# Asunatan/LM-Net

Hardware: AMD Instinct MI355X
Metric: train images/sec at 352x352, 1/2/4/8 MI355X; Dice vs ref (higher is better)
Workload: dtype f32; 1 GPU; LM-Net fp32 training step (fwd + CE/Dice loss + bwd + AdamW), batch 8/GPU, 352x352 synthetic disc masks (BASELINE configs[1]); global_batch=8, parallelism=dp1, launch=lmn_plan_run (recorded C-side schedule, one crossing per pass)

## Files before the change

lm_net_amd/csrc/conv_wgrad.hip:

```cpp
#include "conv_common.h"

namespace {

struct WgradParams {
  LmnLay lay_src[3], lay_dy;
  int32_t rpw;
  uint32_t rp_magic;
  lmn_wgrad_args_t a;
  int ntile_src[3];
  int ntile_off[3];
  int cbase[3];
  int NNTT, NMTT;
  int Cin;
  int nsets_n;
  int steps_per_img;
  int total_steps;
  float inv_keep_src[3];
  float inv_keep_dy;
  float* partial;
  int TH, TW, XH, XW, CSx, CSy, tiles_x, tiles_y, total_tiles;
  uint32_t mXW, mTW;
  int dbg;
};

__device__ __forceinline__ float* wgrad_dst(const WgradParams& P, int co, int sidx, int ch, int taps) {
  float* own = P.a.dW_src[sidx];
  return own ? own + ((int64_t)co * P.a.src[sidx].C + ch) * taps
             : P.a.dW + ((int64_t)co * P.Cin + P.cbase[sidx] + ch) * taps;
}

template <int TAPS, int NMT, int NNT, int PM = 0>
__global__ __launch_bounds__(256, 2) void wgrad_lds_kernel(const WgradParams P) {
  constexpr bool BF = PM >= 1;
  typedef typename ActT<PM>::type TA;
  const lmn_wgrad_args_t& A = P.a;
  const uint32_t soff = A.seed_ctr ? *A.seed_ctr : 0u;
  extern __shared__ __attribute__((aligned(16))) float smem[];
  const int XP = P.XH * P.XW;
  float* XS = smem;
  float* YS = smem + NNT * XP * P.CSx;
  const int tid = threadIdx.x, lane = tid & 63;
  const int wv = __builtin_amdgcn_readfirstlane(tid >> 6);
  const int q = lane >> 4, n = lane & 15;
  const int mset = blockIdx.y / P.nsets_n, nset = blockIdx.y - mset * P.nsets_n;
  const int mt0 = mset * NMT, nt0 = nset * NNT;
  const int pad = A.ksize >> 1;
  const int NP = P.TH * P.TW;

  const TA* tptr[NNT];
  const float* tscale[NNT];
  int tC[NNT], tcs[NNT], tflags[NNT], tch0[NNT];
  uint32_t tseed[NNT];
  float tp_[NNT], tik[NNT];
#pragma unroll
  for (int t = 0; t < NNT; ++t) {
    const int nt = nt0 + t;
    int sidx = 0;
    while (sidx + 1 < A.nsrc && nt >= P.ntile_off[sidx + 1]) ++sidx;
    tptr[t] = (const TA*)A.src[sidx].ptr;
    tscale[t] = A.src[sidx].scale;
    tC[t] = nt < P.NNTT ? A.src[sidx].C : 0;
    tcs[t] = A.src[sidx].cstride;
    tflags[t] = A.src[sidx].flags;
    tseed[t] = A.src[sidx].drop_seed + soff;
    tp_[t] = A.src[sidx].drop_p;
    tik[t] = P.inv_keep_src[sidx];
    tch0[t] = (nt - P.ntile_off[sidx]) * 16;
  }

  f32x4 acc[TAPS][NMT][NNT];
  float bsum[NMT];
#pragma unroll
  for (int tp = 0; tp < TAPS; ++tp)
#pragma unroll
    for (int m = 0; m < NMT; ++m)
#pragma unroll
      for (int t = 0; t < NNT; ++t) acc[tp][m][t] = f32x4{0.f, 0.f, 0.f, 0.f};
#pragma unroll
  for (int m = 0; m < NMT; ++m) bsum[m] = 0.f;

  const int t_begin = (int)(((int64_t)blockIdx.x * P.total_tiles) / gridDim.x);
  const int t_end = (int)(((int64_t)(blockIdx.x + 1) * P.total_tiles) / gridDim.x);
  for (int tile = t_begin; tile < t_end; ++tile) {
    const int b = tile / (P.tiles_x * P.tiles_y), tt = tile - b * P.tiles_x * P.tiles_y;
    const int oy0 = (tt / P.tiles_x) * P.TH, ox0 = (tt % P.tiles_x) * P.TW;
    const int iy0 = oy0 * A.stride - pad, ix0 = ox0 * A.stride - pad;
    __syncthreads();
    constexpr int UX = (TAPS == 9 && NMT * NNT == 4) ? 3 : 4, UY = 2;
    const int NXI = P.XH * P.XW * 4, NYI = NP * 4;
    for (int rd = 0; rd * (UX * 256) < NXI || rd * (UY * 256) < NYI; ++rd) {
      f32x4 vx[UX][NNT], vy[UY][NMT];
      int gpx[UX], gpy[UY];
#pragma unroll
      for (int u = 0; u < UX; ++u) {
        const int i = rd * (UX * 256) + u * 256 + tid;
        const int j = i & 3, pix = i >> 2;
        bool inb;
        int gp;
        if constexpr (TAPS == 1) {
          inb = i < NXI && ox0 + pix < A.Wout;
          gp = inb ? b * A.Wout + ox0 + pix : 0;
        } else {
          const int r = (int)__umulhi((uint32_t)pix, P.mXW), c = pix - r * P.XW;
          const int iy = iy0 + r, ix = ix0 + c;
          inb = i < NXI && (unsigned)iy < (unsigned)A.Hin && (unsigned)ix < (unsigned)A.Win;
          gp = inb ? (b * A.Hin + iy) * A.Win + ix : 0;
// ... 179 lines not shown
            for (int r = 0; r < 4; ++r) {
              float* d = &s_acc[(((tp * NMT + m) * NNT + t) * 4 + r) * 64 + lane];
              *d = (w == 0) ? acc[tp][m][t][r] : *d + acc[tp][m][t][r];
            }
#pragma unroll
      for (int m = 0; m < NMT; ++m) {
        float v = bsum[m];
        v += __shfl_xor(v, 16, 64);
        v += __shfl_xor(v, 32, 64);
        if (q == 0) {
          float* d = &s_acc[NT * 256 + m * 16 + n];
          *d = (w == 0) ? v : *d + v;
        }
      }
    }
    __syncthreads();
  }
  if (P.partial) {
    float* dst = P.partial + ((int64_t)blockIdx.y * gridDim.x + blockIdx.x) * (NT * 256 + NMT * 16);
    for (int i = tid; i < NT * 256 + NMT * 16; i += 256) dst[i] = s_acc[i];
    return;
  }
  for (int i = tid; i < NT * 256; i += 256) {
    const int ln = i & 63, r = (i >> 6) & 3, tl = i >> 8;
    const int t = tl % NNT, m = (tl / NNT) % NMT, tp = tl / (NNT * NMT);
    const int qq = ln >> 4, nn = ln & 15;
    const int co = (mt0 + m) * 16 + qq * 4 + r;
    const int nt = nt0 + t;
    if ((mt0 + m) >= P.NMTT || co >= A.Cout || nt >= P.NNTT) continue;
    int sidx = 0;
    while (sidx + 1 < A.nsrc && nt >= P.ntile_off[sidx + 1]) ++sidx;
    const int ch = (nt - P.ntile_off[sidx]) * 16 + nn;
    if (ch >= A.src[sidx].C) continue;
    atomicAdd(wgrad_dst(P, co, sidx, ch, TAPS) + tp, s_acc[i]);
  }
  if (A.db && nset == 0) {
    for (int i = tid; i < NMT * 16; i += 256) {
      const int co = mt0 * 16 + i;
      if (co < A.Cout && (mt0 + i / 16) < P.NMTT) {
        atomicAdd(A.db + co, s_acc[NT * 256 + i]);
        if (A.db2) atomicAdd(A.db2 + co, s_acc[NT * 256 + i]);
      }
    }
  }
}

template <int ESZ> struct RawOf { typedef f32x4 type; };
template <> struct RawOf<2> { typedef u32x2 type; };
__device__ __forceinline__ f32x4 raw_f32(f32x4 v) { return v; }
__device__ __forceinline__ f32x4 raw_f32(u32x2 v) { return f32x4{lmn_bf16_lo(v.x), lmn_bf16_hi(v.x), lmn_bf16_lo(v.y), lmn_bf16_hi(v.y)}; }
template <typename RawT> __device__ __forceinline__ RawT raw_load(BufRsrc r, uint32_t off) {
  if constexpr (sizeof(RawT) == 16) return __builtin_bit_cast(f32x4, __builtin_amdgcn_raw_buffer_load_b128(r, (int)off, 0, 0));
  else return __builtin_amdgcn_raw_buffer_load_b64(r, (int)off, 0, 0);
}
#ifdef LMN_WG_TIMING
__device__ unsigned long long g_wg_timing[4096 * 6];
#define LMN_TCLK() __builtin_amdgcn_s_memtime()
#endif

template <int NMT, int NNT, int PM, bool UP = false>
__global__ __launch_bounds__(256, 3) void wgrad3_kernel(const WgradParams P) {
  static_assert(NMT * NNT == 4 || NMT * NNT == 1, "one-tile or 2 x 2-tile blocks");
  constexpr bool TS = NMT * NNT == 4;
  constexpr bool BF = PM >= 1;
  typedef typename ActT<PM>::type TA;
  constexpr int ESZ = sizeof(TA);
  typedef typename RawOf<ESZ>::type RawT;
  constexpr int XWC = 34, CS = BF ? 12 : 16;
  constexpr int QW = BF ? 2 : 4;
  constexpr int UX = TS ? 4 : 6, UY = TS ? 2 : 4;
  constexpr int XPA = UX * 64, NPA = UY * 64;
  const lmn_wgrad_args_t& A = P.a;
  const uint32_t soff = A.seed_ctr ? *A.seed_ctr : 0u;
  extern __shared__ __attribute__((aligned(16))) float smem[];
  float* XS = smem;
  float* YS = smem + NNT * XPA * CS;
  constexpr int USX = TS ? 2 : 3;
  constexpr int SCW = 19, SPA = USX * 64;
  float* S2 = YS + NMT * NPA * CS;
  (void)S2;
  const int tid = threadIdx.x, lane = tid & 63;
  const int wv = __builtin_amdgcn_readfirstlane(tid >> 6);
  const int q = lane >> 4, n = lane & 15;
  const int m_w = TS ? wv / NNT : 0, t_w = TS ? wv % NNT : 0;
  const int mset = blockIdx.y / P.nsets_n, nset = blockIdx.y - mset * P.nsets_n;
  const int mt0 = mset * NMT, nt0 = nset * NNT;
  const int NP = P.TH * 32;
  const int j = tid & 3, pl = tid >> 2;

  const float* tscale[NNT];
  int tC[NNT], tcs[NNT], tflags[NNT], tch0[NNT];
  uint32_t tseed[NNT];
  float tp_[NNT], tik[NNT];
  BufRsrc rx[NNT];
  bool cx[NNT];
#pragma unroll
  for (int t = 0; t < NNT; ++t) {
    const int nt = nt0 + t;
    int sidx = 0;
    while (sidx + 1 < A.nsrc && nt >= P.ntile_off[sidx + 1]) ++sidx;
    tscale[t] = A.src[sidx].scale;
    tC[t] = nt < P.NNTT ? A.src[sidx].C : 0;
    tcs[t] = A.src[sidx].cstride;
    tflags[t] = A.src[sidx].flags;
    tseed[t] = A.src[sidx].drop_seed + soff;
    tp_[t] = A.src[sidx].drop_p;
    tik[t] = P.inv_keep_src[sidx];
    tch0[t] = (nt - P.ntile_off[sidx]) * 16;
    rx[t] = make_rsrc(A.src[sidx].ptr, (unsigned)((int64_t)A.B * (UP ? (A.Hin >> 1) * (A.Win >> 1) : A.Hin * A.Win) * tcs[t] * ESZ));
    cx[t] = tch0[t] + j * 4 < tC[t];
  }
  const BufRsrc ry = make_rsrc(A.dy, (unsigned)((int64_t)A.B * A.Hout * A.Wout * A.dy_cstride * ESZ));

  uint32_t xrc[UX], xo[UX][NNT];
#pragma unroll
  for (int u = 0; u < UX; ++u) {
    const int pix = u * 64 + pl, r = pix / XWC, c = pix - r * XWC;
    xrc[u] = r < P.XH ? (uint32_t)(r << 16 | c) : 0x7fff0000u;
#pragma unroll
    for (int t = 0; t < NNT; ++t) xo[u][t] = (uint32_t)(((r * A.Win + c) * tcs[t] + tch0[t] + j * 4) * ESZ);
  }
  const int yc = pl & 31, yr0 = pl >> 5;
  uint32_t yo0[NMT];
  bool cy[NMT];
#pragma unroll
  for (int m = 0; m < NMT; ++m) {
    const int co = (mt0 + m) * 16 + j * 4;
    cy[m] = (mt0 + m) < P.NMTT && co < A.Cout;
    yo0[m] = (uint32_t)(((yr0 * A.Wout + yc) * A.dy_cstride + (cy[m] ? co : 0)) * ESZ);
  }
  const uint32_t ystep = (uint32_t)(2 * A.Wout * A.dy_cstride * ESZ);

  f32x4 acc[9];
  float bsum = 0.f;
#pragma unroll
  for (int tp = 0; tp < 9; ++tp) acc[tp] = f32x4{0.f, 0.f, 0.f, 0.f};

  RawT vx[UP ? 1 : UX][NNT], vy[UY][NMT];
  RawT vs[UP ? USX : 1][NNT];
  const int tpi = P.tiles_x * P.tiles_y;
  const int hs = A.Hin >> 1, ws = A.Win >> 1;
  const float up_sh = UP ? (float)(hs - 1) / (float)(A.Hin - 1) : 0.f, up_sw = UP ? (float)(ws - 1) / (float)(A.Win - 1) : 0.f;
  auto src_org = [&](int iy0, int ix0, int& ys0, int& xs0) __attribute__((always_inline)) {
    ys0 = (int)(up_sh * (float)(iy0 > 0 ? iy0 : 0));
    xs0 = (int)(up_sw * (float)(ix0 > 0 ? ix0 : 0));
  };
  auto issue = [&](int tile) __attribute__((always_inline)) {
    const int b = tile / tpi, tt = tile - b * tpi;
    const int ty_ = tt / P.tiles_x;
    const int oy0 = ty_ * P.TH, ox0 = (tt - ty_ * P.tiles_x) * 32;
    const int iy0 = oy0 - 1, ix0 = ox0 - 1;
    const int wpix = (b * A.Hin + iy0) * A.Win + ix0;
    if constexpr (UP) {
      int ys0, xs0;
      src_org(iy0, ix0, ys0, xs0);
#pragma unroll
      for (int u = 0; u < USX; ++u) {
        const int sp = u * 64 + pl, sr = sp / SCW, sc = sp - sr * SCW;
        const bool inb = ys0 + sr < hs && xs0 + sc < ws;
#pragma unroll
        for (int t = 0; t < NNT; ++t) {
          const uint32_t off = (uint32_t)((((b * hs + ys0 + sr) * ws + xs0 + sc) * tcs[t] + tch0[t] + j * 4) * ESZ);
          vs[u][t] = raw_load<RawT>(rx[t], (inb && cx[t]) ? off : 0xffffffffu);
        }
      }
    } else {
#pragma unroll
    for (int u = 0; u < UX; ++u) {
      const int r = (int)(xrc[u] >> 16), c = (int)(xrc[u] & 0xffffu);
      const bool inb = (unsigned)(iy0 + r) < (unsigned)A.Hin && (unsigned)(ix0 + c) < (unsigned)A.Win;
#pragma unroll
      for (int t = 0; t < NNT; ++t) {
        const uint32_t off = (uint32_t)(wpix * tcs[t] * ESZ) + xo[u][t];
        vx[u][t] = raw_load<RawT>(rx[t], (inb && cx[t]) ? off : 0xffffffffu);
      }
    }
    }
    const uint32_t ybase = (uint32_t)(((b * A.Hout + oy0) * A.Wout + ox0) * A.dy_cstride * ESZ);
    const bool cok = ox0 + yc < A.Wout;
    const int rlim = (A.Hout - oy0 < P.TH ? A.Hout - oy0 : P.TH) - yr0;
#pragma unroll
    for (int u = 0; u < UY; ++u) {
      const bool inb = cok && 2 * u < rlim;
#pragma unroll
      for (int m = 0; m < NMT; ++m)
        vy[u][m] = raw_load<RawT>(ry, (inb && cy[m]) ? ybase + (uint32_t)u * ystep + yo0[m] : 0xffffffffu);
    }
  };
  float* xl = XS + pl * CS + j * QW;
  float* yl = YS + pl * CS + j * QW;
  auto commit = [&](int tile) __attribute__((always_inline)) {
    const int b = tile / tpi, tt = tile - b * tpi;
    const int ty_ = tt / P.tiles_x;
    const int oy0 = ty_ * P.TH, ox0 = (tt - ty_ * P.tiles_x) * 32;
    if constexpr (UP) {
#pragma unroll
      for (int t = 0; t < NNT; ++t)
#pragma unroll
        for (int u = 0; u < USX; ++u) *reinterpret_cast<f32x4*>(&S2[((t * SPA) + u * 64 + pl) * 16 + j * 4]) = raw_f32(vs[u][t]);
      __syncthreads();
      const int iy0 = oy0 - 1, ix0 = ox0 - 1;
      int ys0, xs0;
      src_org(iy0, ix0, ys0, xs0);
#pragma unroll
      for (int u = 0; u < UX; ++u) {
        const int r = (int)(xrc[u] >> 16), c = (int)(xrc[u] & 0xffffu);
        const int iy = iy0 + r, ix = ix0 + c;
        const bool inb = (unsigned)iy < (unsigned)A.Hin && (unsigned)ix < (unsigned)A.Win;
        int y0, yp, x0, xp;
        float ly0, ly1, lx0, lx1;
        lmn_up_coord(inb ? iy : 0, hs, up_sh, y0, yp, ly0, ly1);
        lmn_up_coord(inb ? ix : 0, ws, up_sw, x0, xp, lx0, lx1);
        const int l00 = inb ? (y0 - ys0) * SCW + (x0 - xs0) : 0;
#pragma unroll
        for (int t = 0; t < NNT; ++t) {
          const float* sp = &S2[(t * SPA + l00) * 16 + j * 4];
          const f32x4 v00 = *reinterpret_cast<const f32x4*>(sp), v01 = *reinterpret_cast<const f32x4*>(sp + xp * 16);
          const f32x4 v10 = *reinterpret_cast<const f32x4*>(sp + yp * SCW * 16), v11 = *reinterpret_cast<const f32x4*>(sp + (yp * SCW + xp) * 16);
          f32x4 w = ly0 * (lx0 * v00 + lx1 * v01) + ly1 * (lx0 * v10 + lx1 * v11);
          if (!inb) w = f32x4{0.f, 0.f, 0.f, 0.f};
          float* dst = xl + (t * XPA + u * 64) * CS;
          if constexpr (BF) *reinterpret_cast<uint2*>(dst) = pk4_bf16(w);
          else *reinterpret_cast<f32x4*>(dst) = w;
        }
      }
    } else {
#pragma unroll
    for (int t = 0; t < NNT; ++t) {
      const bool tf = tflags[t] != 0 || tscale[t] != nullptr;
#pragma unroll
      for (int u = 0; u < UX; ++u) {
        float* dst = xl + (t * XPA + u * 64) * CS;
        if (!tf) {
          if constexpr (ESZ == 2) *reinterpret_cast<u32x2*>(dst) = vx[u][t];
          else if constexpr (BF) *reinterpret_cast<uint2*>(dst) = pk4_bf16(raw_f32(vx[u][t]));
          else *reinterpret_cast<f32x4*>(dst) = raw_f32(vx[u][t]);
          continue;
        }
        f32x4 w = raw_f32(vx[u][t]);
        const int chs = cx[t] ? tch0[t] + j * 4 : 0;
        if (tflags[t] & LMN_SRC_GELU) {
#pragma unroll
          for (int k = 0; k < 4; ++k) w[k] = lmn_gelu(w[k]);
        }
        if (tflags[t] & LMN_SRC_DROP) {
          const int r = (int)(xrc[u] >> 16), c = (int)(xrc[u] & 0xffffu);
          const int gp = (b * A.Hin + oy0 - 1 + r) * A.Win + ox0 - 1 + c;
#pragma unroll
          for (int k = 0; k < 4; ++k) w[k] *= lmn_drop_scale(tseed[t], (uint32_t)(gp * tC[t] + chs + k), tp_[t], tik[t]);
        }
        if (tscale[t]) w *= ld4(tscale[t] + b * tC[t] + chs);
        if constexpr (BF) *reinterpret_cast<uint2*>(dst) = pk4_bf16(w);
        else *reinterpret_cast<f32x4*>(dst) = w;
      }
    }
    }
#pragma unroll
    for (int m = 0; m < NMT; ++m) {
#pragma unroll
      for (int u = 0; u < UY; ++u) {
        float* dst = yl + (m * NPA + u * 64) * CS;
        if (!(A.dy_flags & LMN_SRC_DROP)) {
          if constexpr (ESZ == 2) *reinterpret_cast<u32x2*>(dst) = vy[u][m];
          else if constexpr (BF) *reinterpret_cast<uint2*>(dst) = pk4_bf16(raw_f32(vy[u][m]));
          else *reinterpret_cast<f32x4*>(dst) = raw_f32(vy[u][m]);
          continue;
        }
        f32x4 w = raw_f32(vy[u][m]);
        const int cos = cy[m] ? (mt0 + m) * 16 + j * 4 : 0;
        const int gp = (b * A.Hout + oy0 + 2 * u + yr0) * A.Wout + ox0 + yc;
#pragma unroll
        for (int k = 0; k < 4; ++k) w[k] *= lmn_drop_scale(A.dy_seed + soff, (uint32_t)(gp * A.Cout + cos + k), A.dy_p, P.inv_keep_dy);
        if constexpr (BF) *reinterpret_cast<uint2*>(dst) = pk4_bf16(w);
        else *reinterpret_cast<f32x4*>(dst) = w;
      }
    }
  };

  const int t_begin = (int)(((int64_t)blockIdx.x * P.total_tiles) / gridDim.x);
  const int t_end = (int)(((int64_t)(blockIdx.x + 1) * P.total_tiles) / gridDim.x);
#ifdef LMN_WG_TIMING
  unsigned long long tk0 = LMN_TCLK(), tk_s1 = 0, tk_s2 = 0, tk_s3 = 0, tk_a, tk_b;
#endif
  if (t_begin < t_end) issue(t_begin);
  const int K0 = TS ? 0 : wv, KSTEP = TS ? 1 : 4;
  for (int tile = t_begin; tile < t_end; ++tile) {
#ifdef LMN_WG_TIMING
    tk_a = LMN_TCLK();
#endif
    __syncthreads();
#ifdef LMN_WG_TIMING
    tk_b = LMN_TCLK(); tk_s1 += tk_b - tk_a; tk_a = tk_b;
#endif
    commit(tile);
#ifdef LMN_WG_TIMING
    __builtin_amdgcn_s_waitcnt(0);
    tk_b = LMN_TCLK(); tk_s2 += tk_b - tk_a; tk_a = tk_b;
#endif
    __syncthreads();
    if (tile + 1 < t_end) issue(tile + 1);
#ifdef LMN_WG_TIMING
    tk_b = LMN_TCLK(); tk_s3 += tk_b - tk_a;
#endif
    if constexpr (BF) {
      const uint16_t* xw = reinterpret_cast<const uint16_t*>(XS) + (t_w * XPA + q * 4) * (CS * 2) + n;
      const uint16_t* yw = reinterpret_cast<const uint16_t*>(YS) + (m_w * NPA + q * 4) * (CS * 2) + n;
      auto kfrag = [&](int ks, uint2& av, uint2 (&bv)[9]) __attribute__((always_inline)) {
        const int pix0 = ks * 16, pr = pix0 >> 5, pc0 = pix0 & 31;
        const uint16_t* xp = xw + (pr * XWC + pc0) * (CS * 2);
        const uint16_t* yp = yw + pix0 * (CS * 2);
        uint32_t h[4];
#pragma unroll
        for (int jj = 0; jj < 4; ++jj) {
          h[jj] = yp[jj * CS * 2];
          bsum += __builtin_bit_cast(float, h[jj] << 16);
        }
        av = uint2{h[0] | (h[1] << 16), h[2] | (h[3] << 16)};
#pragma unroll
        for (int tp = 0; tp < 9; ++tp) {
          const uint16_t* xt = xp + ((tp / 3) * XWC + tp % 3) * (CS * 2);
          const uint32_t h0 = xt[0], h1 = xt[CS * 2], h2 = xt[2 * CS * 2], h3 = xt[3 * CS * 2];
          bv[tp] = uint2{h0 | (h1 << 16), h2 | (h3 << 16)};
        }
      };
      int ks = K0;
      for (; (ks + KSTEP) * 16 < NP; ks += 2 * KSTEP) {
        uint2 av0, av1, bv0[9], bv1[9];
        kfrag(ks, av0, bv0);
        kfrag(ks + KSTEP, av1, bv1);
#pragma unroll
        for (int tp = 0; tp < 9; ++tp) acc[tp] = mfma_bf16x2(av0, av1, bv0[tp], bv1[tp], acc[tp]);
      }
      if (ks * 16 < NP) {
        uint2 av, bv[9];
        kfrag(ks, av, bv);
#pragma unroll
        for (int tp = 0; tp < 9; ++tp) acc[tp] = mfma_bf16(av, bv[tp], acc[tp]);
      }
    } else {
      const float* xw = XS + (t_w * XPA + q) * CS + n;
      const float* yw = YS + (m_w * NPA + q) * CS + n;
      for (int ks = K0; ks * 4 < NP; ks += KSTEP) {
        const int pix0 = ks * 4, pr = pix0 >> 5, pc0 = pix0 & 31;
        const float* xp = xw + (pr * XWC + pc0) * CS;
        const float av = yw[pix0 * CS];
        float bv[9];
#pragma unroll
        for (int tp = 0; tp < 9; ++tp) bv[tp] = xp[((tp / 3) * XWC + tp % 3) * CS];
        bsum += av;
#pragma unroll
        for (int tp = 0; tp < 9; ++tp) acc[tp] = __builtin_amdgcn_mfma_f32_16x16x4f32(av, bv[tp], acc[tp], 0, 0, 0);
      }
    }
  }
#ifdef LMN_WG_TIMING
  {
    const unsigned long long tk_e = LMN_TCLK();
    const int bid = blockIdx.y * gridDim.x + blockIdx.x;
    if (tid == 0 && bid < 4096) {
      g_wg_timing[bid * 6 + 0] = tk_s1;
      g_wg_timing[bid * 6 + 1] = tk_s2;
      g_wg_timing[bid * 6 + 2] = tk_s3;
      g_wg_timing[bid * 6 + 3] = tk_e - tk0 - tk_s1 - tk_s2 - tk_s3;
      g_wg_timing[bid * 6 + 4] = tk0;
      g_wg_timing[bid * 6 + 5] = tk_e;
    }
  }
#endif

  constexpr int NT = 9 * NMT * NNT;
  float* pdst = P.partial ? P.partial + ((int64_t)blockIdx.y * gridDim.x + blockIdx.x) * (NT * 256 + NMT * 16) : nullptr;
  if constexpr (TS) {
    const int nt = nt0 + t_w;
    int sidx = 0;
    while (sidx + 1 < A.nsrc && nt >= P.ntile_off[sidx + 1]) ++sidx;
    const int ch = (nt - P.ntile_off[sidx]) * 16 + n;
#pragma unroll
    for (int tp = 0; tp < 9; ++tp)
#pragma unroll
      for (int r = 0; r < 4; ++r) {
        if (pdst) {
          pdst[(((tp * NMT + m_w) * NNT + t_w) * 4 + r) * 64 + lane] = acc[tp][r];
        } else {
          const int co = (mt0 + m_w) * 16 + q * 4 + r;
          if ((mt0 + m_w) < P.NMTT && co < A.Cout && nt < P.NNTT && ch < A.src[sidx].C)
            atomicAdd(wgrad_dst(P, co, sidx, ch, 9) + tp, acc[tp][r]);
        }
      }
    if (t_w == 0) {
      float v = bsum;
      v += __shfl_xor(v, 16, 64);
      v += __shfl_xor(v, 32, 64);
      if (q == 0) {
        const int co = (mt0 + m_w) * 16 + n;
        if (pdst) pdst[NT * 256 + m_w * 16 + n] = v;
        else if (A.db && nset == 0 && co < A.Cout && (mt0 + m_w) < P.NMTT) {
          atomicAdd(A.db + co, v);
          if (A.db2) atomicAdd(A.db2 + co, v);
        }
      }
    }
    return;
  }
  __syncthreads();
  float* s_acc = smem;
  for (int w = 0; w < 4; ++w) {
    if (wv == w) {
#pragma unroll
      for (int tp = 0; tp < 9; ++tp)
#pragma unroll
        for (int r = 0; r < 4; ++r) {
          float* d = &s_acc[(tp * 4 + r) * 64 + lane];
          *d = (w == 0) ? acc[tp][r] : *d + acc[tp][r];
        }
      float v = bsum;
      v += __shfl_xor(v, 16, 64);
      v += __shfl_xor(v, 32, 64);
      if (q == 0) {
        float* d = &s_acc[NT * 256 + n];
        *d = (w == 0) ? v : *d + v;
      }
    }
    __syncthreads();
  }
  if (pdst) {
    for (int i = tid; i < NT * 256 + 16; i += 256) pdst[i] = s_acc[i];
    return;
  }
  for (int i = tid; i < NT * 256; i += 256) {
    const int ln = i & 63, r = (i >> 6) & 3, tp = i >> 8;
    const int co = mt0 * 16 + (ln >> 4) * 4 + r;
    if (mt0 >= P.NMTT || co >= A.Cout || nt0 >= P.NNTT) continue;
    int sidx = 0;
    while (sidx + 1 < A.nsrc && nt0 >= P.ntile_off[sidx + 1]) ++sidx;
    const int ch = (nt0 - P.ntile_off[sidx]) * 16 + (ln & 15);
    if (ch >= A.src[sidx].C) continue;
    atomicAdd(wgrad_dst(P, co, sidx, ch, 9) + tp, s_acc[i]);
  }
  if (A.db && nset == 0 && tid < 16) {
    const int co = mt0 * 16 + tid;
    if (co < A.Cout && mt0 < P.NMTT) {
      atomicAdd(A.db + co, s_acc[NT * 256 + tid]);
      if (A.db2) atomicAdd(A.db2 + co, s_acc[NT * 256 + tid]);
    }
  }
}

template <int NMT, int NNT, int PM = 0>
__global__ __launch_bounds__(256) void wgrad_1x1_kernel(const WgradParams P) {
  constexpr int PMB = PM & 3;
  constexpr bool RP = (PM & 4) != 0;
  constexpr bool BF = PMB >= 1;
  typedef typename ActT<PMB>::type TA;
  constexpr int U = 8;
  const lmn_wgrad_args_t& A = P.a;
  const uint32_t soff = A.seed_ctr ? *A.seed_ctr : 0u;
  const int lane = threadIdx.x & 63;
  const int q = lane >> 4, n = lane & 15;
  const int wvb = __builtin_amdgcn_readfirstlane(threadIdx.x >> 6);
  const int wave = blockIdx.x * 4 + wvb, nwaves = gridDim.x * 4;
  const int mset = blockIdx.y / P.nsets_n, nset = blockIdx.y - mset * P.nsets_n;
  const int mt0 = mset * NMT, nt0 = nset * NNT;
  const int HW = A.Hout * A.Wout;
  const int NPX = A.B * HW;

  const TA* sptr[NNT];
  const float* sscale[NNT];
  int sC[NNT], scs[NNT], sflags[NNT], sch[NNT];
  uint32_t scho[NNT], srf[NNT];
  uint32_t sseed[NNT];
  float sp[NNT], sik[NNT];
  bool any_tf = (A.dy_flags & LMN_SRC_DROP) != 0;
// ... 468 lines not shown
  const int mt0 = mset * NMT, nt0 = nset * NNT;
  const float* src = J.partial + (int64_t)set * nblk * PER;
  const int epq = 1024 / ksl, epb = epq * 4;
  const int q = threadIdx.x & (epq - 1), ks = threadIdx.x / epq;
  const int i4 = (bx * epq + q) * 4;
  f32x4 s4 = f32x4{0.f, 0.f, 0.f, 0.f};
  if (i4 < PER) {
    const float* sp = src + i4;
#pragma unroll 4
    for (int k = ks; k < nblk; k += ksl) s4 += *reinterpret_cast<const f32x4*>(sp + (int64_t)k * PER);
  }
  *reinterpret_cast<f32x4*>(&red[threadIdx.x * 4]) = s4;
  __syncthreads();
  for (int e = threadIdx.x; e < epb; e += 1024) {
    const int i = bx * epb + e;
    if (i >= PER) return;
    float sum = 0.f;
    for (int k = 0; k < ksl; ++k) sum += red[k * epb + e];
    if (i < NT * 256) {
      const int ln = i & 63, r = (i >> 6) & 3, tile = i >> 8;
      const int t = tile % NNT, m = (tile / NNT) % NMT, tp = tile / (NNT * NMT);
      const int qq = ln >> 4, nn = ln & 15;
      const int co = (mt0 + m) * 16 + qq * 4 + r;
      const int nt = nt0 + t;
      if ((mt0 + m) >= J.NMTT || co >= J.Cout || nt >= J.NNTT) continue;
      int sidx = 0;
      while (sidx + 1 < J.nsrc && nt >= J.ntile_off[sidx + 1]) ++sidx;
      const int ch = (nt - J.ntile_off[sidx]) * 16 + nn;
      if (ch >= J.srcC[sidx]) continue;
      float* own = J.dW_src[sidx];
      float* d = own ? own + ((int64_t)co * J.srcC[sidx] + ch) * TAPS : J.dW + ((int64_t)co * J.Cin + J.cbase[sidx] + ch) * TAPS;
      d[tp] += sum;
    } else if (J.db && nset == 0) {
      const int j = i - NT * 256, co = mt0 * 16 + j;
      if (co < J.Cout && (mt0 + j / 16) < J.NMTT) {
        J.db[co] += sum;
        if (J.db2) J.db2[co] += sum;
      }
    }
  }
}

}

template <int M, int N, int PM>
static void wgrad3_launch(dim3 grid, size_t shmem, hipStream_t st, const WgradParams& P) {
  if constexpr (M * N == 4 || M * N == 1) {
    if (P.a.src[0].flags & LMN_SRC_UP2) LMN_LAUNCH((wgrad3_kernel<M, N, PM, true>), grid, dim3(256), shmem, st, P);
    else LMN_LAUNCH((wgrad3_kernel<M, N, PM>), grid, dim3(256), shmem, st, P);
  }
}

extern "C" {

int lmn_sizeof_wgrad_args(void) { return (int)sizeof(lmn_wgrad_args_t); }

static void wgrad_tile_shape(const lmn_wgrad_args_t& a, int nmtt, int nntt, int* NMT, int* NNT) {
  bool rp_any = a.dy_rp_w != 0;
  for (int s = 0; s < a.nsrc && s < 3; ++s) rp_any = rp_any || a.src[s].rp_w != 0 || (a.src[s].flags & LMN_SRC_LN) != 0;
  const bool direct = a.ksize == 1 && a.stride == 1 && ((int64_t)a.Hout * a.Wout >= 32 || rp_any);
  if (direct) {
    static const int shapes[][2] = {{1, 1}, {1, 2}, {1, 3}, {1, 4}, {2, 1}, {3, 1}, {4, 1}, {2, 2}, {2, 3}, {3, 2}, {2, 4}, {4, 2}};
    int cin = 0;
    for (int s = 0; s < a.nsrc && s < 3; ++s) cin += a.src[s].C;
    long best = -1;
    for (const auto& sh : shapes) {
      const int M = sh[0], N = sh[1];
      if (M > nmtt && M > 1) continue;
      if (N > nntt && N > 1) continue;
      const long cost = ((long)((nmtt + M - 1) / M) * cin + (long)((nntt + N - 1) / N) * a.Cout) * 64 + M * N;
      if (best < 0 || cost < best) { best = cost; *NMT = M; *NNT = N; }
    }
    return;
  }
  const bool small = nmtt == 1 || nntt == 1;
  *NMT = small ? 1 : 2; *NNT = small ? 1 : 2;
}

static int wgrad_v1_env() {
  static int v = -1;
  if (v < 0) { const char* e = getenv("LMN_WGRAD_V1"); v = e ? atoi(e) : 1; }
  return v;
}
static bool wgrad_v1(const lmn_wgrad_args_t& a) { return a.ksize == 3 && a.stride == 1 && wgrad_v1_env() != 0; }
static int wgrad_blocks_total(const lmn_wgrad_args_t& a) {
  static int c = -1;
  if (c < 0) { const char* e = getenv("LMN_WGRAD_CAP"); c = e ? atoi(e) : 0; }
  if (!wgrad_v1(a)) return 512;
  return c > 0 ? c : 512;
}

int64_t lmn_conv_wgrad_workspace(const lmn_wgrad_args_t* a) {
  if (!a) return 0;
  int nntt = 0;
  for (int s = 0; s < a->nsrc && s < 3; ++s) nntt += (a->src[s].C + 15) / 16;
  const int nmtt = (a->Cout + 15) / 16;
  int NMT, NNT;
  wgrad_tile_shape(*a, nmtt, nntt, &NMT, &NNT);
  const int gy = ((nmtt + NMT - 1) / NMT) * ((nntt + NNT - 1) / NNT);
  const int64_t per = (int64_t)a->ksize * a->ksize * NMT * NNT * 256 + NMT * 16;
  const int btot = wgrad_blocks_total(*a);
  const int64_t cap = btot / gy > 2 ? btot / gy : 2;
  const int64_t need = gy * cap * per;
  return need <= (int64_t)(16 << 20) ? need : 0;
}
#ifdef LMN_WG_TIMING
int lmn_wg_timing(unsigned long long* out, int n) {
  return (int)hipMemcpyFromSymbol(out, HIP_SYMBOL(g_wg_timing), sizeof(unsigned long long) * n);
}
#endif

static int reduce_slices(int nblk) {
  int k = 1;
  while (k < 64 && k * 4 < nblk) k <<= 1;
  return k;
}

static bool wgrad_two_stage(int64_t gy, int64_t blocks, int64_t per) {
  return blocks > 48 || gy * blocks * per > 256 * 1024;
}

struct WgGeom {
  int NMT, NNT, gy, taps, blocks;
  int64_t per;
  bool direct, v1, wave_staged;
  size_t shmem;
  int pm;
};

static int wgrad_setup(const lmn_wgrad_args_t& A, WgradParams& P, WgGeom& G) {
  LMN_REQUIRE(A.ksize == 1 || A.ksize == 3, "conv_wgrad: ksize %d", A.ksize);
  LMN_REQUIRE(A.stride == 1 || A.stride == 2, "conv_wgrad: stride %d", A.stride);
  LMN_REQUIRE(A.nsrc >= 1 && A.nsrc <= 3, "conv_wgrad: nsrc %d", A.nsrc);
  LMN_REQUIRE(A.dy && A.Cout > 0 && A.dy_cstride >= A.Cout, "conv_wgrad: dy/Cout");
  for (int s = 0; s < A.nsrc && s < 3; ++s) LMN_REQUIRE(A.dW || A.dW_src[s], "conv_wgrad: no gradient tensor for source %d", s);
  LMN_REQUIRE(!A.db2 || A.db, "conv_wgrad: db2 without db");
  LMN_REQUIRE(A.B > 0 && A.Hout > 0 && A.Wout > 0, "conv_wgrad: empty tensor");
  LMN_REQUIRE(A.mma_dtype == LMN_F32 || A.mma_dtype == LMN_BF16, "conv_wgrad: mma_dtype %d", A.mma_dtype);
  LMN_REQUIRE(A.act_dtype == LMN_F32 || (A.act_dtype == LMN_BF16 && A.mma_dtype == LMN_BF16),
              "conv_wgrad: act_dtype %d with mma_dtype %d", A.act_dtype, A.mma_dtype);
  P.a = A;
  P.NNTT = 0;
  P.Cin = 0;
  for (int s = 0; s < 3; ++s) {
    P.ntile_src[s] = P.ntile_off[s] = P.cbase[s] = 0;
    P.inv_keep_src[s] = 1.f;
  }
  for (int s = 0; s < A.nsrc; ++s) {
    LMN_REQUIRE(A.src[s].ptr && A.src[s].C > 0 && A.src[s].cstride >= A.src[s].C, "conv_wgrad: source %d", s);
    P.ntile_src[s] = (A.src[s].C + 15) / 16;
    P.ntile_off[s] = P.NNTT;
    P.cbase[s] = P.Cin;
    P.NNTT += P.ntile_src[s];
    P.Cin += A.src[s].C;
    if (A.src[s].flags & LMN_SRC_DROP) P.inv_keep_src[s] = 1.f / (1.f - A.src[s].drop_p);
  }
  P.inv_keep_dy = (A.dy_flags & LMN_SRC_DROP) ? 1.f / (1.f - A.dy_p) : 1.f;
  {
    int rw = 0;
    for (int s = 0; s < 3; ++s) {
      const int w = s < A.nsrc ? A.src[s].rp_w : 0;
      P.lay_src[s] = lmn_lay_make(w, s < A.nsrc ? A.src[s].C : 4, s < A.nsrc ? A.src[s].cstride : 4);
      if (w) {
        LMN_REQUIRE(w > 0 && A.src[s].cstride == A.src[s].C && (rw == 0 || rw == w), "conv_wgrad: row-planar source %d must be a whole tensor (cstride == C) of the call's width", s);
        rw = w;
      }
    }
    P.lay_dy = lmn_lay_make(A.dy_rp_w, A.Cout, A.dy_cstride);
    if (A.dy_rp_w) { LMN_REQUIRE(A.dy_rp_w > 0 && A.dy_cstride == A.Cout && (rw == 0 || rw == A.dy_rp_w), "conv_wgrad: row-planar dy must be a whole tensor of the call's width"); rw = A.dy_rp_w; }
    if (rw) LMN_REQUIRE(A.ksize == 1 && A.stride == 1 && rw == A.Wout && rw == A.Win, "conv_wgrad: row-planar operands belong to 1x1 stride-1 calls over images of their own width (rp_w %d, call %d)", rw, A.Wout);
    P.rpw = rw;
    P.rp_magic = lmn_div_magic(rw);
  }
  P.NMTT = (A.Cout + 15) / 16;
  P.steps_per_img = (A.Hout * A.Wout + 3) / 4;
  LMN_REQUIRE((int64_t)A.B * P.steps_per_img < (1LL << 31), "conv_wgrad: too many pixels");
  for (int s = 0; s < A.nsrc; ++s)
    LMN_REQUIRE((int64_t)A.B * A.Hin * A.Win * A.src[s].cstride < (1LL << 31), "conv_wgrad: source %d larger than 2^31 elements", s);
  LMN_REQUIRE((int64_t)A.B * A.Hout * A.Wout * A.dy_cstride < (1LL << 31), "conv_wgrad: dy larger than 2^31 elements");
  P.total_steps = A.B * P.steps_per_img;
  if (A.ksize == 1 && A.stride == 1) {
    P.a.Wout = A.Hout * A.Wout; P.a.Hout = 1;
    P.a.Win = A.Hin * A.Win; P.a.Hin = 1;
  }
  int NMT, NNT;
  wgrad_tile_shape(A, P.NMTT, P.NNTT, &NMT, &NNT);
  const int msets = (P.NMTT + NMT - 1) / NMT;
  P.nsets_n = (P.NNTT + NNT - 1) / NNT;
  const int gy = msets * P.nsets_n;
  const int taps = A.ksize * A.ksize;
  const int64_t per = (int64_t)taps * NMT * NNT * 256 + NMT * 16;
  const lmn_wgrad_args_t& Gm = P.a;
  const bool v1c = wgrad_v1(A) && Gm.Wout >= 32 && (NMT * NNT == 4 || NMT * NNT == 1);
  const int npmax = Gm.stride == 2 ? 64 : ((Gm.ksize == 1 || NMT * NNT == 1 || (Gm.Wout <= 32 && !v1c)) ? 256 : 128);
  P.TW = Gm.Wout < (Gm.ksize == 1 ? npmax : 32) ? Gm.Wout : (Gm.ksize == 1 ? npmax : 32);
  if (Gm.stride == 2 && P.TW > 16) P.TW = 16;
  P.TH = npmax / P.TW;
  if (P.TH > Gm.Hout) P.TH = Gm.Hout;
  if (P.TH < 1) P.TH = 1;
  P.XH = (P.TH - 1) * Gm.stride + Gm.ksize;
  P.XW = (P.TW - 1) * Gm.stride + Gm.ksize;
  P.CSy = 16;
  P.CSx = A.stride == 1 ? 16 : 24;
  const bool bf = A.mma_dtype == LMN_BF16;
  const int pm = bf ? (A.act_dtype == LMN_BF16 ? 2 : 1) : 0;
  if (bf) P.CSy = P.CSx = 12;
  P.tiles_x = (Gm.Wout + P.TW - 1) / P.TW;
  P.tiles_y = (Gm.Hout + P.TH - 1) / P.TH;
  P.total_tiles = A.B * P.tiles_x * P.tiles_y;
  P.dbg = 0;
  LMN_REQUIRE(P.XH * P.XW < 65536 && P.TH * P.TW < 65536, "conv_wgrad: tile too large");
  P.mXW = (uint32_t)((1ull << 32) / (uint32_t)P.XW + 1);
  P.mTW = (uint32_t)((1ull << 32) / (uint32_t)P.TW + 1);
  int64_t lds_floats = (int64_t)NNT * P.XH * P.XW * P.CSx + (int64_t)NMT * P.TH * P.TW * P.CSy;
  if (lds_floats < per) lds_floats = per;
  LMN_REQUIRE(lds_floats * 4 <= 160 * 1024, "conv_wgrad: LDS tile too large (%lld B)", (long long)lds_floats * 4);
  int64_t blocks64 = P.total_tiles;
  const int64_t esz = A.act_dtype == LMN_BF16 ? 2 : 4;
  bool v1 = v1c && P.TW == 32 && P.XW == 34 &&
            P.XH * P.XW * 4 <= (NMT * NNT == 1 ? 6 : 4) * 256 && P.TH * P.TW * 4 <= (NMT * NNT == 1 ? 4 : 2) * 256 &&
            (int64_t)A.B * A.Hout * A.Wout * A.dy_cstride * esz < 0xfffffff0LL;
  for (int s = 0; s < A.nsrc; ++s) v1 = v1 && (int64_t)A.B * A.Hin * A.Win * A.src[s].cstride * esz < 0xfffffff0LL;
  bool up2 = false;
  for (int s = 0; s < A.nsrc; ++s) up2 = up2 || (A.src[s].flags & LMN_SRC_UP2) != 0;
  if (v1) {
    const int ux = NMT * NNT == 1 ? 6 : 4, uy = NMT * NNT == 1 ? 4 : 2, cs = bf ? 12 : 16;
    lds_floats = (int64_t)(NNT * ux + NMT * uy) * 64 * cs;
    if (up2) lds_floats += (int64_t)NNT * (NMT * NNT == 1 ? 3 : 2) * 64 * 16;
    if (NMT * NNT == 1 && lds_floats < per) lds_floats = per;
  }
  if (up2) {
    LMN_REQUIRE(A.nsrc == 1 && A.ksize == 3 && A.stride == 1 && A.Hin % 2 == 0 && A.Win % 2 == 0 && !(A.src[0].flags & ~LMN_SRC_UP2) && !A.src[0].scale,
                "conv_wgrad: LMN_SRC_UP2 belongs to single-source 3x3 stride-1 calls (Hin x Win = the upsampled size) without other source transforms");
    int64_t big = (int64_t)A.B * A.Hout * A.Wout * A.dy_cstride * esz;
    const int64_t xb = (int64_t)A.B * A.Hin * A.Win * A.src[0].cstride * esz;
    if (xb > big) big = xb;
    LMN_REQUIRE(big < 0xfffffff0LL,
                "conv_wgrad: LMN_SRC_UP2: an operand of %lld bytes (counted at the upsampled size) is not below the 4294967280-byte limit of the wgrad3 "
                "form's 32-bit byte offsets: upsample with lmn_up2_fwd and take the plain weight gradient (lmn_conv_wgrad_up2_ok says so beforehand)",
                (long long)big);
    LMN_REQUIRE(v1 && (P.XH + 1) / 2 + 2 <= (NMT * NNT == 1 ? 3 : 2) * 64 / 19,
                "conv_wgrad: LMN_SRC_UP2 needs the wgrad3 form (upsampled map >= 32 wide; lmn_conv_wgrad_up2_ok says so beforehand)");
  }
  static int cap_other = -1;
  if (cap_other < 0) { const char* e = getenv("LMN_WGRAD_CAP_OTHER"); cap_other = e && atoi(e) > 0 ? atoi(e) : 512; }
  const int btot = v1 ? wgrad_blocks_total(A) : cap_other;
  const int64_t cap = btot / gy > 2 ? btot / gy : 2;
  if (blocks64 > cap) blocks64 = cap;
  if (blocks64 < 1) blocks64 = 1;
  bool rp_any = A.dy_rp_w != 0, ln_any = false;
  for (int s = 0; s < A.nsrc; ++s) { rp_any = rp_any || A.src[s].rp_w != 0; ln_any = ln_any || (A.src[s].flags & LMN_SRC_LN) != 0; }
  G.direct = A.ksize == 1 && A.stride == 1 && ((int64_t)Gm.Hout * Gm.Wout >= 32 || rp_any || ln_any);
  if (G.direct) {
    const int64_t steps = ((int64_t)A.B * Gm.Hout * Gm.Wout + 3) / 4;
    blocks64 = (steps + 63) / 64;
    if (blocks64 > cap) blocks64 = cap;
    if (blocks64 < 1) blocks64 = 1;
  }
  P.partial = nullptr;
  if (A.workspace && (wgrad_two_stage(gy, blocks64, per) || (g_lmn_det && blocks64 > 1)) && (int64_t)gy * blocks64 * per <= A.workspace_floats) {
    P.partial = A.workspace;
  } else if (g_lmn_det) {
    blocks64 = 1;
  } else if (blocks64 > 512 / gy && 512 / gy >= 2) {
    blocks64 = 512 / gy;
  }
  G.NMT = NMT; G.NNT = NNT; G.gy = gy; G.taps = taps; G.per = per; G.blocks = (int)blocks64;
  G.v1 = v1; G.pm = pm; G.shmem = (size_t)lds_floats * 4;
  bool any_tf = (A.dy_flags & LMN_SRC_DROP) != 0;
  for (int s = 0; s < A.nsrc; ++s) any_tf = any_tf || A.src[s].flags != 0 || A.src[s].scale != nullptr;
  const bool old_shape = (NMT == 1 && NNT <= 4) || (NNT == 1 && NMT <= 4) || (NMT == 2 && NNT == 2);
  G.wave_staged = !(pm == 2 && !any_tf && old_shape) || (rp_any && (int64_t)Gm.Hout * Gm.Wout < 32);
  for (int s = 0; s < A.nsrc; ++s) {
    if (A.src[s].flags & LMN_SRC_LN) {
      LMN_REQUIRE(A.nsrc == 1 && G.direct && G.wave_staged && !rp_any, "conv_wgrad: LMN_SRC_LN belongs to single-source NHWC 1x1 stride-1 calls");
      LMN_REQUIRE(A.src[s].ln_gamma && A.src[s].ln_beta && A.src[s].ln_stats, "conv_wgrad: LMN_SRC_LN needs ln_gamma / ln_beta and the ln_stats table of the forward conv");
      LMN_REQUIRE(!(A.src[s].flags & ~LMN_SRC_LN) && !A.src[s].scale, "conv_wgrad: LMN_SRC_LN does not combine with other source transforms");
    }
  }
  return 0;
}

int lmn_sizeof_reduce_job(void) { return (int)sizeof(lmn_reduce_job_t); }

int lmn_conv_wgrad_up2_ok(const lmn_wgrad_args_t* args) {
  if (!args || args->nsrc != 1 || args->ksize != 3 || args->stride != 1 || (args->Hin & 1) || (args->Win & 1)) return 0;
  if ((args->src[0].flags & ~LMN_SRC_UP2) || args->src[0].scale) return 0;
  lmn_wgrad_args_t a = *args;
  a.src[0].flags = 0;
  WgradParams P;
  WgGeom G;
  char keep[sizeof(g_lmn_err)];
  memcpy(keep, g_lmn_err, sizeof(keep));
// ... 158 lines not shown
```

Baseline: 597.7 images/sec.

## Split wgrad taps across idle waves when 2x2 tile set is partially out of range

In the 2x2 wave-tiled wgrad kernel, blocks at the edge of the Cout or Cin tile grid used to leave waves working on nonexistent tiles. Now those waves share the 9 filter taps of the valid tile, split 5/4 or 3/3/3, and skip staging the missing tiles into LDS. The intent is to shorten the critical path of edge blocks so the last blocks finish sooner. In exchange it adds templated kloop variants, which increases code size and register pressure, and extra branching in the staging and output paths. It is gated by LMN_WGRAD_FILL, which defaults to on.

```diff
diff --git a/lm_net_amd/csrc/conv_wgrad.hip b/lm_net_amd/csrc/conv_wgrad.hip
--- a/lm_net_amd/csrc/conv_wgrad.hip
+++ b/lm_net_amd/csrc/conv_wgrad.hip
@@ -21,7 +21,9 @@
   int TH, TW, XH, XW, CSx, CSy, tiles_x, tiles_y, total_tiles;
   uint32_t mXW, mTW;
   int dbg;
+  int fill;
 };
+template <int V> struct WgIC { static constexpr int value = V; };
 
 __device__ __forceinline__ float* wgrad_dst(const WgradParams& P, int co, int sidx, int ch, int taps) {
   float* own = P.a.dW_src[sidx];
@@ -367,9 +369,15 @@
   const int tid = threadIdx.x, lane = tid & 63;
   const int wv = __builtin_amdgcn_readfirstlane(tid >> 6);
   const int q = lane >> 4, n = lane & 15;
-  const int m_w = TS ? wv / NNT : 0, t_w = TS ? wv % NNT : 0;
   const int mset = blockIdx.y / P.nsets_n, nset = blockIdx.y - mset * P.nsets_n;
   const int mt0 = mset * NMT, nt0 = nset * NNT;
+  const bool vr2 = TS && (!P.fill || mt0 + 1 < P.NMTT), vc2 = TS && (!P.fill || nt0 + 1 < P.NNTT);
+  const int m_w = vr2 ? wv >> 1 : 0, t_w = vc2 ? wv & 1 : 0;
+  const int nshare = TS ? (vr2 ? 1 : 2) * (vc2 ? 1 : 2) : 1;
+  const int rank = TS ? (vc2 ? 0 : wv & 1) + (vr2 ? 0 : wv >> 1) * (vc2 ? 1 : 2) : 0;
+  const int TP0 = nshare == 2 ? rank * 5 : (nshare == 4 ? rank * 3 : 0);
+  const int TPN = nshare == 2 ? 5 - rank : (nshare == 4 ? (rank < 3 ? 3 : 0) : 9);
+  const int trow = nshare == 4 && rank < 3 ? rank : 0;
   const int NP = P.TH * 32;
   const int j = tid & 3, pl = tid >> 2;
 
@@ -480,9 +488,11 @@
     const int oy0 = ty_ * P.TH, ox0 = (tt - ty_ * P.tiles_x) * 32;
     if constexpr (UP) {
 #pragma unroll
-      for (int t = 0; t < NNT; ++t)
+      for (int t = 0; t < NNT; ++t) {
+        if (t > 0 && !vc2) continue;
 #pragma unroll
         for (int u = 0; u < USX; ++u) *reinterpret_cast<f32x4*>(&S2[((t * SPA) + u * 64 + pl) * 16 + j * 4]) = raw_f32(vs[u][t]);
+      }
       __syncthreads();
       const int iy0 = oy0 - 1, ix0 = ox0 - 1;
       int ys0, xs0;
@@ -499,6 +509,7 @@
         const int l00 = inb ? (y0 - ys0) * SCW + (x0 - xs0) : 0;
 #pragma unroll
         for (int t = 0; t < NNT; ++t) {
+          if (t > 0 && !vc2) continue;
           const float* sp = &S2[(t * SPA + l00) * 16 + j * 4];
           const f32x4 v00 = *reinterpret_cast<const f32x4*>(sp), v01 = *reinterpret_cast<const f32x4*>(sp + xp * 16);
           const f32x4 v10 = *reinterpret_cast<const f32x4*>(sp + yp * SCW * 16), v11 = *reinterpret_cast<const f32x4*>(sp + (yp * SCW + xp) * 16);
@@ -512,6 +523,7 @@
     } else {
 #pragma unroll
     for (int t = 0; t < NNT; ++t) {
+      if (t > 0 && !vc2) continue;
       const bool tf = tflags[t] != 0 || tscale[t] != nullptr;
 #pragma unroll
       for (int u = 0; u < UX; ++u) {
@@ -542,6 +554,7 @@
     }
 #pragma unroll
     for (int m = 0; m < NMT; ++m) {
+      if (m > 0 && !vr2) continue;
 #pragma unroll
       for (int u = 0; u < UY; ++u) {
         float* dst = yl + (m * NPA + u * 64) * CS;
@@ -587,10 +600,13 @@
 #ifdef LMN_WG_TIMING
     tk_b = LMN_TCLK(); tk_s3 += tk_b - tk_a;
 #endif
+    auto kloop = [&](auto tpfc, auto ntpc) __attribute__((always_inline)) {
+    constexpr int TPF = decltype(tpfc)::value, NTP = decltype(ntpc)::value;
+    auto tapoff = [&](int i) __attribute__((always_inline)) { return ((TPF + i) / 3) * XWC + (TPF + i) % 3; };
     if constexpr (BF) {
-      const uint16_t* xw = reinterpret_cast<const uint16_t*>(XS) + (t_w * XPA + q * 4) * (CS * 2) + n;
+      const uint16_t* xw = reinterpret_cast<const uint16_t*>(XS) + (t_w * XPA + trow * XWC + q * 4) * (CS * 2) + n;
       const uint16_t* yw = reinterpret_cast<const uint16_t*>(YS) + (m_w * NPA + q * 4) * (CS * 2) + n;
-      auto kfrag = [&](int ks, uint2& av, uint2 (&bv)[9]) __attribute__((always_inline)) {
+      auto kfrag = [&](int ks, uint2& av, uint2 (&bv)[NTP]) __attribute__((always_inline)) {
         const int pix0 = ks * 16, pr = pix0 >> 5, pc0 = pix0 & 31;
         const uint16_t* xp = xw + (pr * XWC + pc0) * (CS * 2);
         const uint16_t* yp = yw + pix0 * (CS * 2);
@@ -602,40 +618,52 @@
         }
         av = uint2{h[0] | (h[1] << 16), h[2] | (h[3] << 16)};
 #pragma unroll
-        for (int tp = 0; tp < 9; ++tp) {
-          const uint16_t* xt = xp + ((tp / 3) * XWC + tp % 3) * (CS * 2);
+        for (int tp = 0; tp < NTP; ++tp) {
+          const uint16_t* xt = xp + tapoff(tp) * (CS * 2);
           const uint32_t h0 = xt[0], h1 = xt[CS * 2], h2 = xt[2 * CS * 2], h3 = xt[3 * CS * 2];
           bv[tp] = uint2{h0 | (h1 << 16), h2 | (h3 << 16)};
         }
       };
       int ks = K0;
       for (; (ks + KSTEP) * 16 < NP; ks += 2 * KSTEP) {
-        uint2 av0, av1, bv0[9], bv1[9];
+        uint2 av0, av1, bv0[NTP], bv1[NTP];
         kfrag(ks, av0, bv0);
         kfrag(ks + KSTEP, av1, bv1);
 #pragma unroll
-        for (int tp = 0; tp < 9; ++tp) acc[tp] = mfma_bf16x2(av0, av1, bv0[tp], bv1[tp], acc[tp]);
+        for (int tp = 0; tp < NTP; ++tp)
+          acc[tp] = mfma_bf16x2(av0, av1, bv0[tp], bv1[tp], acc[tp]);
       }
       if (ks * 16 < NP) {
-        uint2 av, bv[9];
+        uint2 av, bv[NTP];
         kfrag(ks, av, bv);
 #pragma unroll
-        for (int tp = 0; tp < 9; ++tp) acc[tp] = mfma_bf16(av, bv[tp], acc[tp]);
+        for (int tp = 0; tp < NTP; ++tp)
+          acc[tp] = mfma_bf16(av, bv[tp], acc[tp]);
       }
     } else {
-      const float* xw = XS + (t_w * XPA + q) * CS + n;
+      const float* xw = XS + (t_w * XPA + trow * XWC + q) * CS + n;
       const float* yw = YS + (m_w * NPA + q) * CS + n;
       for (int ks = K0; ks * 4 < NP; ks += KSTEP) {
         const int pix0 = ks * 4, pr = pix0 >> 5, pc0 = pix0 & 31;
         const float* xp = xw + (pr * XWC + pc0) * CS;
         const float av = yw[pix0 * CS];
-        float bv[9];
-#pragma unroll
-        for (int tp = 0; tp < 9; ++tp) bv[tp] = xp[((tp / 3) * XWC + tp % 3) * CS];
+        float bv[NTP];
+#pragma unroll
+        for (int tp = 0; tp < NTP; ++tp) bv[tp] = xp[tapoff(tp) * CS];
         bsum += av;
 #pragma unroll
-        for (int tp = 0; tp < 9; ++tp) acc[tp] = __builtin_amdgcn_mfma_f32_16x16x4f32(av, bv[tp], acc[tp], 0, 0, 0);
-      }
+        for (int tp = 0; tp < NTP; ++tp)
+          acc[tp] = __builtin_amdgcn_mfma_f32_16x16x4f32(av, bv[tp], acc[tp], 0, 0, 0);
+      }
+    }
+    };
+    if constexpr (TS) {
+      if (nshare == 1) kloop(WgIC<0>(), WgIC<9>());
+      else if (nshare == 2 && rank == 0) kloop(WgIC<0>(), WgIC<5>());
+      else if (nshare == 2) kloop(WgIC<5>(), WgIC<4>());
+      else if (rank < 3) kloop(WgIC<0>(), WgIC<3>());
+    } else {
+      kloop(WgIC<0>(), WgIC<9>());
     }
   }
 #ifdef LMN_WG_TIMING
@@ -661,18 +689,22 @@
     while (sidx + 1 < A.nsrc && nt >= P.ntile_off[sidx + 1]) ++sidx;
     const int ch = (nt - P.ntile_off[sidx]) * 16 + n;
 #pragma unroll
-    for (int tp = 0; tp < 9; ++tp)
-#pragma unroll
-      for (int r = 0; r < 4; ++r) {
-        if (pdst) {
-          pdst[(((tp * NMT + m_w) * NNT + t_w) * 4 + r) * 64 + lane] = acc[tp][r];
-        } else {
-          const int co = (mt0 + m_w) * 16 + q * 4 + r;
-          if ((mt0 + m_w) < P.NMTT && co < A.Cout && nt < P.NNTT && ch < A.src[sidx].C)
-            atomicAdd(wgrad_dst(P, co, sidx, ch, 9) + tp, acc[tp][r]);
-        }
-      }
-    if (t_w == 0) {
+    for (int i = 0; i < 9; ++i) {
+      const int tp = TP0 + i;
+      if (i < TPN) {
+#pragma unroll
+        for (int r = 0; r < 4; ++r) {
+          if (pdst) {
+            pdst[(((tp * NMT + m_w) * NNT + t_w) * 4 + r) * 64 + lane] = acc[i][r];
+          } else {
+            const int co = (mt0 + m_w) * 16 + q * 4 + r;
+            if ((mt0 + m_w) < P.NMTT && co < A.Cout && nt < P.NNTT && ch < A.src[sidx].C)
+              atomicAdd(wgrad_dst(P, co, sidx, ch, 9) + tp, acc[i][r]);
+          }
+        }
+      }
+    }
+    if (t_w == 0 && rank == 0) {
       float v = bsum;
       v += __shfl_xor(v, 16, 64);
       v += __shfl_xor(v, 32, 64);
@@ -1307,6 +1339,11 @@
   if (v < 0) { const char* e = getenv("LMN_WGRAD_V1"); v = e ? atoi(e) : 1; }
   return v;
 }
+static int wgrad_fill_env() {
+  static int v = -1;
+  if (v < 0) { const char* e = getenv("LMN_WGRAD_FILL"); v = e ? (atoi(e) != 0) : 1; }
+  return v;
+}
 static bool wgrad_v1(const lmn_wgrad_args_t& a) { return a.ksize == 3 && a.stride == 1 && wgrad_v1_env() != 0; }
 static int wgrad_blocks_total(const lmn_wgrad_args_t& a) {
   static int c = -1;
@@ -1434,6 +1471,7 @@
   P.tiles_y = (Gm.Hout + P.TH - 1) / P.TH;
   P.total_tiles = A.B * P.tiles_x * P.tiles_y;
   P.dbg = 0;
+  P.fill = wgrad_fill_env();
   LMN_REQUIRE(P.XH * P.XW < 65536 && P.TH * P.TW < 65536, "conv_wgrad: tile too large");
   P.mXW = (uint32_t)((1ull << 32) / (uint32_t)P.XW + 1);
   P.mTW = (uint32_t)((1ull << 32) / (uint32_t)P.TW + 1);
```

Result: faster. 604.9 images/sec (median of 6 runs) (+1.2%).
